# qcraftai/gedepth

Measured on AMD Instinct MI355X. Metric: training img/s (whole node), KITTI-shaped 352x1120 synthetic batches, higher is better.
Workload: dtype bf16; 1 GPU; depthformer_swint_v: DepthFormer-SwinT + GEDepth-Vanilla, 352x1120, 8 img/GPU, full train step; global_batch=8, parallelism=dp1, allreduce_dtype=fp32, layout=nhwc, window_attention=bf16 mfma, params=53516992, hip_graph=off

## Files before the change

gedepth_amd/csrc/conv3x3_wgrad.hip:

```cpp
#include "common.h"

#define WG_TH 8
#define WG_TW 32
#define WG_HALO ((WG_TH + 2) * (WG_TW + 2))
#define WG_PIX (WG_TH * WG_TW)
#define WG_DY_PIECES (WG_PIX * 8)
#define WG_X_PIECES (WG_HALO * 4)

template <int TAP0, int NTAP>
__device__ __forceinline__ void wg_tile_mfma(const bf16_t* dyh, const bf16_t* xt, ge_f32x16* acc) {
  ge_bf16x8 A[2], B[2][NTAP];
#define WG_RD(P) __builtin_shufflevector(__builtin_amdgcn_ds_read_tr16_b64_v4bf16(GE_LDS(ge_bf16x4, (P))), \
                                         __builtin_amdgcn_ds_read_tr16_b64_v4bf16(GE_LDS(ge_bf16x4, (P) + 4 * 32)), 0, 1, 2, 3, 4, 5, 6, 7)
#define WG_FRAGS(SET, KS)                                                                                   \
  {                                                                                                         \
    constexpr int row_ = (KS) >> 1, xh_ = ((KS) & 1) * 16;                                                  \
    A[SET] = WG_RD(dyh + (row_ * 32 + xh_) * 32);                                                           \
    _Pragma("unroll") for (int j = 0; j < NTAP; ++j) {                                                     \
      const int r_ = (TAP0 + j) / 3, s_ = (TAP0 + j) - 3 * r_;                                              \
      B[SET][j] = WG_RD(xt + ((row_ + r_) * (WG_TW + 2) + xh_ + s_) * 32);                                  \
    }                                                                                                       \
  }
#define WG_STEP(KS)                                                                                         \
  {                                                                                                         \
    if ((KS) < 15) WG_FRAGS(((KS) + 1) & 1, ((KS) + 1) & 15)                                                \
    __builtin_amdgcn_sched_barrier(0);                                                                      \
    _Pragma("unroll") for (int j = 0; j < NTAP; ++j)                                                       \
      acc[j] = __builtin_amdgcn_mfma_f32_32x32x16_bf16(A[(KS) & 1], B[(KS) & 1][j], acc[j], 0, 0, 0);       \
    __builtin_amdgcn_sched_barrier(0);                                                                      \
  }
  WG_FRAGS(0, 0)
  WG_STEP(0) WG_STEP(1) WG_STEP(2) WG_STEP(3) WG_STEP(4) WG_STEP(5) WG_STEP(6) WG_STEP(7)
  WG_STEP(8) WG_STEP(9) WG_STEP(10) WG_STEP(11) WG_STEP(12) WG_STEP(13) WG_STEP(14) WG_STEP(15)
#undef WG_STEP
#undef WG_FRAGS
#undef WG_RD
}

__global__ void __launch_bounds__(256, 2) conv3x3_wgrad_k(const bf16_t* __restrict__ x, const bf16_t* __restrict__ dy, float* __restrict__ dw, int N, int H,
                                                          int W, int Cin, int Cout, int tiles_x, int tiles_y, int ksplit) {
  __shared__ __attribute__((aligned(16))) bf16_t dy_t[2 * WG_PIX * 32];
  __shared__ __attribute__((aligned(16))) bf16_t x_t[WG_HALO * 32];
  const int tid = threadIdx.x, lane = tid & 63, wv = tid >> 6;
  const int c0 = blockIdx.x * 32, n0 = blockIdx.y * 64;
  const int mb = wv & 1, tap0 = (wv >> 1) ? 5 : 0, ntap = (wv >> 1) ? 4 : 5;
  ge_f32x16 acc[5];
#pragma unroll
  for (int t = 0; t < 5; ++t) acc[t] = 0.f;
  const int tr_pix = (lane >> 5) * 8 + ((lane & 15) >> 2), tr_col = ((lane >> 4) & 1) * 16 + (lane & 3) * 4;
  const int total_tiles = N * tiles_y * tiles_x;
  uint4 pd[8], px[6];
  const uint4 zero4 = make_uint4(0, 0, 0, 0);
  int dy_yx[8], dy_lds[8], x_yx[6], x_lds[6];
  const int dy_ch = n0 + (tid & 7) * 8, x_ch = c0 + (tid & 3) * 8;
#pragma unroll
  for (int i = 0; i < 8; ++i) {
    const int p = tid + i * 256, pix = p >> 3, part = p & 7;
    dy_yx[i] = ((pix >> 5) << 16) | (pix & 31);
    dy_lds[i] = ((part >> 2) * WG_PIX + pix) * 32 + (part & 3) * 8;
  }
#pragma unroll
  for (int i = 0; i < 6; ++i) {
    const int p = tid + i * 256, pix = p >> 2;
    const int iy = pix / (WG_TW + 2), ix = pix - iy * (WG_TW + 2);
    x_yx[i] = p < WG_X_PIECES ? ((iy << 16) | ix) : -1;
    x_lds[i] = (p >> 2) * 32 + (p & 3) * 8;
  }
  const bool dy_ch_ok = dy_ch < Cout;
#define WG_PREFETCH(T)                                                                                       \
  {                                                                                                          \
    const int t_ = __builtin_amdgcn_readfirstlane(T);                                                        \
    const int per_img = tiles_y * tiles_x;                                                                   \
    const int n_ = t_ / per_img, rem_ = t_ - n_ * per_img;                                                   \
    const int tyi = rem_ / tiles_x;                                                                          \
    const int ty0 = tyi * WG_TH, tx0 = (rem_ - tyi * tiles_x) * WG_TW;                                       \
    const bf16_t* dyn = dy + (long)n_ * H * W * Cout + dy_ch;                                                \
    const bf16_t* xn = x + (long)n_ * H * W * Cin + x_ch;                                                    \
    _Pragma("unroll") for (int i = 0; i < 8; ++i) {                                                         \
      const int gy = ty0 + (dy_yx[i] >> 16), gx = tx0 + (dy_yx[i] & 0xffff);                                 \
      pd[i] = zero4;                                                                                         \
      if (gy < H && gx < W && dy_ch_ok) pd[i] = *(const uint4*)(dyn + (gy * W + gx) * Cout);                 \
    }                                                                                                        \
    _Pragma("unroll") for (int i = 0; i < 6; ++i) {                                                         \
      const int gy = ty0 + (x_yx[i] >> 16) - 1, gx = tx0 + (x_yx[i] & 0xffff) - 1;                           \
      px[i] = zero4;                                                                                         \
      if (x_yx[i] >= 0 && gy >= 0 && gy < H && gx >= 0 && gx < W) px[i] = *(const uint4*)(xn + (gy * W + gx) * Cin); \
    }                                                                                                        \
  }
#define WG_PARK()                                                                                            \
  _Pragma("unroll") for (int i = 0; i < 8; ++i) *(uint4*)(dy_t + dy_lds[i]) = pd[i];                        \
  _Pragma("unroll") for (int i = 0; i < 6; ++i) {                                                           \
    if (x_yx[i] >= 0) *(uint4*)(x_t + x_lds[i]) = px[i];                                                     \
  }
  int t = blockIdx.z;
  if (t < total_tiles) {
    WG_PREFETCH(t)
    WG_PARK()
  }
  __syncthreads();
  for (; t < total_tiles; t += ksplit) {
    const bool more = t + ksplit < total_tiles;
    if (more) { WG_PREFETCH(t + ksplit) }
    const bf16_t* dyh = dy_t + mb * WG_PIX * 32 + tr_pix * 32 + tr_col;
    const bf16_t* xt = x_t + tr_pix * 32 + tr_col;
    if (wv >> 1) wg_tile_mfma<5, 4>(dyh, xt, acc);
    else wg_tile_mfma<0, 5>(dyh, xt, acc);
    __syncthreads();
    if (more) { WG_PARK() }
    __syncthreads();
  }
#undef WG_PREFETCH
#undef WG_PARK
  const int ci = c0 + (lane & 31);
#pragma unroll
  for (int j = 0; j < 5; ++j) {
    if (j < ntap) {
      const int tap = tap0 + j;
#pragma unroll
      for (int r = 0; r < 16; ++r) {
        const int co = n0 + mb * 32 + (r & 3) + 8 * (r >> 2) + 4 * (lane >> 5);
        if (co < Cout) atomicAdd(dw + ((long)co * 9 + tap) * Cin + ci, acc[j][r]);
      }
    }
  }
}

extern "C" int ge_conv3x3_nhwc_wgrad(const void* x, const void* dy, float* dw, int N, int H, int W, int Cin, int Cout, int dtype, void* stream) {
  if (!x || !dy || !dw || N < 0 || H <= 0 || W <= 0 || Cin <= 0 || Cout <= 0) return GE_ERR_BAD_ARG;
  if (dtype != GE_BF16 || Cin % 32 || Cout % 8 || (((uintptr_t)x | (uintptr_t)dy) & 15)) return GE_ERR_UNSUPPORTED;
  if (N == 0) return GE_OK;
  const int tiles_x = (W + WG_TW - 1) / WG_TW, tiles_y = (H + WG_TH - 1) / WG_TH;
  const long total = (long)N * tiles_y * tiles_x;
  if (total >= (1L << 31) || (long)H * W * std::max(Cin, Cout) >= (1L << 31)) return GE_ERR_UNSUPPORTED;
  const int blocks_out = (Cin / 32) * ((Cout + 63) / 64);
  const int cus = ge_cu_count();
  if (!cus) return GE_ERR_BAD_ARG;
  long ksplit = (2L * cus) / blocks_out;
  if (ksplit > total) ksplit = total;
  if (ksplit < 1) ksplit = 1;
  if (ksplit > 65535 || (Cout + 63) / 64 > 65535) return GE_ERR_UNSUPPORTED;
  const dim3 grid(Cin / 32, (Cout + 63) / 64, (unsigned)ksplit);
  conv3x3_wgrad_k<<<grid, 256, 0, ge_stream(stream)>>>((const bf16_t*)x, (const bf16_t*)dy, dw, N, H, W, Cin, Cout, tiles_x, tiles_y, (int)ksplit);
  GE_LAUNCH_CHECK();
  return GE_OK;
}
```

Baseline: 171.4 img/s.

## Rewrite conv3x3 wgrad with direct global-to-LDS DMA interleaved into MFMA loop

Replaces the register-staged prefetch/park wgrad kernel with a 512-thread kernel. Each block covers 64 input and 64 output channels and fills double-buffered LDS using global_load_lds_dwordx4, issued one slot per MFMA step so loads overlap compute. Work is split across waves by tap-role, blocks are remapped for XCD locality, and the per-class k-split is chosen from a cost table. This removes the VGPR staging and the second barrier, but adds large LDS use (160KB, one block per CU), inline asm, and more complex indexing. Only the conv3x3 weight gradient inside the full train step is affected.

```diff
diff --git a/gedepth_amd/csrc/conv3x3_wgrad.hip b/gedepth_amd/csrc/conv3x3_wgrad.hip
--- a/gedepth_amd/csrc/conv3x3_wgrad.hip
+++ b/gedepth_amd/csrc/conv3x3_wgrad.hip
@@ -4,11 +4,9 @@
 #define WG_TW 32
 #define WG_HALO ((WG_TH + 2) * (WG_TW + 2))
 #define WG_PIX (WG_TH * WG_TW)
-#define WG_DY_PIECES (WG_PIX * 8)
-#define WG_X_PIECES (WG_HALO * 4)
 
-template <int TAP0, int NTAP>
-__device__ __forceinline__ void wg_tile_mfma(const bf16_t* dyh, const bf16_t* xt, ge_f32x16* acc) {
+template <int TAP0, int NTAP, typename D>
+__device__ __forceinline__ void wg_tile_mfma(const bf16_t* dyh, const bf16_t* xt, ge_f32x16* acc, D&& dma) {
   ge_bf16x8 A[2], B[2][NTAP];
 #define WG_RD(P) __builtin_shufflevector(__builtin_amdgcn_ds_read_tr16_b64_v4bf16(GE_LDS(ge_bf16x4, (P))), \
                                          __builtin_amdgcn_ds_read_tr16_b64_v4bf16(GE_LDS(ge_bf16x4, (P) + 4 * 32)), 0, 1, 2, 3, 4, 5, 6, 7)
@@ -25,6 +23,7 @@
   {                                                                                                         \
     if ((KS) < 15) WG_FRAGS(((KS) + 1) & 1, ((KS) + 1) & 15)                                                \
     __builtin_amdgcn_sched_barrier(0);                                                                      \
+    dma(KS);                                                                                                \
     _Pragma("unroll") for (int j = 0; j < NTAP; ++j)                                                       \
       acc[j] = __builtin_amdgcn_mfma_f32_32x32x16_bf16(A[(KS) & 1], B[(KS) & 1][j], acc[j], 0, 0, 0);       \
     __builtin_amdgcn_sched_barrier(0);                                                                      \
@@ -37,81 +36,123 @@
 #undef WG_RD
 }
 
-__global__ void __launch_bounds__(256, 2) conv3x3_wgrad_k(const bf16_t* __restrict__ x, const bf16_t* __restrict__ dy, float* __restrict__ dw, int N, int H,
-                                                          int W, int Cin, int Cout, int tiles_x, int tiles_y, int ksplit) {
-  __shared__ __attribute__((aligned(16))) bf16_t dy_t[2 * WG_PIX * 32];
-  __shared__ __attribute__((aligned(16))) bf16_t x_t[WG_HALO * 32];
-  const int tid = threadIdx.x, lane = tid & 63, wv = tid >> 6;
-  const int c0 = blockIdx.x * 32, n0 = blockIdx.y * 64;
-  const int mb = wv & 1, tap0 = (wv >> 1) ? 5 : 0, ntap = (wv >> 1) ? 4 : 5;
+#define WD_XSLAB (22 * 1024)
+#define WD_XOFF (2 * WG_PIX * 64)
+#define WD_NPIECE (32 + 2 * 22)
+#define WD_SLOTS 10
+#define WD_BUF (80 * 1024)
+#ifndef WD_COST
+#define WD_COST {16, 11, 11, 7}
+#endif
+
+__device__ __attribute__((aligned(16))) uint32_t wd_zero16[4] = {0, 0, 0, 0};
+
+struct WdSplit { int k[4]; };
+
+__global__ void __launch_bounds__(512, 1) conv3x3_wgrad_dma_k(const bf16_t* __restrict__ x, const bf16_t* __restrict__ dy, float* __restrict__ dw, int N,
+                                                              int H, int W, int Cin, int Cout, int tiles_x, int tiles_y, WdSplit ks) {
+  __shared__ __attribute__((aligned(1024))) unsigned char smem[2 * WD_BUF];
+  const int tid = threadIdx.x, lane = tid & 63;
+  const int wv = __builtin_amdgcn_readfirstlane(tid >> 6);
+  const int chunks = Cin >> 5, pf = chunks >> 1, tail = chunks & 1;
+  const int cbs = (Cout + 63) >> 6, half = (Cout - 64 * (cbs - 1)) <= 32 ? 1 : 0, cf = cbs - half;
+  int b, pair, cb, ksplit;
+  {
+    const int per = gridDim.x >> 3, rem = gridDim.x & 7, xcd = blockIdx.x & 7;
+    b = xcd * per + (xcd < rem ? xcd : rem) + (blockIdx.x >> 3);
+  }
+  const int cnt0 = pf * cf * ks.k[0], cnt1 = pf * half * ks.k[1], cnt2 = tail * cf * ks.k[2];
+  if (b < cnt0) { ksplit = ks.k[0]; const int nb = pf * cf, z = b / nb, blk = b - z * nb; pair = blk / cf; cb = blk - pair * cf; b = z; }
+  else if ((b -= cnt0) < cnt1) { ksplit = ks.k[1]; const int z = b / pf; pair = b - z * pf; cb = cf; b = z; }
+  else if ((b -= cnt1) < cnt2) { ksplit = ks.k[2]; const int z = b / cf; cb = b - z * cf; pair = pf; b = z; }
+  else { b -= cnt2; ksplit = ks.k[3]; pair = pf; cb = cf; }
+  const int c0 = pair * 64, n0 = cb * 64;
+  const int nh = n0 + 32 < Cout ? 2 : 1, nc = c0 + 32 < Cin ? 2 : 1, units = nh * nc;
+  const int total_tiles = N * tiles_y * tiles_x, per_img = tiles_y * tiles_x;
+  int t = b;
+  if (t >= total_tiles) return;
+  int mb, ch, role;
+  if (units == 4) { ch = wv & 1; mb = wv >> 2; role = ((wv >> 1) & 1) ^ mb; }
+  else {
+    const int u = wv >> 2;
+    mb = nh == 2 ? u : 0; ch = nc == 2 ? u : 0;
+    role = u < units ? 2 + ((wv + 2 * u) & 3) : -1;
+  }
+  const int tap0 = role == 1 ? 5 : role == 3 ? 3 : role == 4 ? 5 : role == 5 ? 7 : 0;
+  const int ntap = role < 0 ? 0 : role == 0 ? 5 : role == 1 ? 4 : role == 2 ? 3 : 2;
   ge_f32x16 acc[5];
 #pragma unroll
-  for (int t = 0; t < 5; ++t) acc[t] = 0.f;
+  for (int j = 0; j < 5; ++j) acc[j] = 0.f;
+
+  int yx[WD_SLOTS];
+  const unsigned part16 = (lane & 3) * 16;
+#pragma unroll
+  for (int i = 0; i < WD_SLOTS; ++i) {
+    const int p = wv + 8 * i;
+    int v = -1;
+    if (p < 32) {
+      const int pix = (p & 15) * 16 + (lane >> 2);
+      if (n0 + (p >> 4) * 32 + (lane & 3) * 8 < Cout) v = (((pix >> 5) + 1) << 16) | ((pix & 31) + 1);
+    } else if (p < WD_NPIECE) {
+      const int q = p - 32, c = q >= 22 ? 1 : 0, hp = (q - 22 * c) * 16 + (lane >> 2);
+      if (hp < WG_HALO && c < nc) { const int iy = hp / (WG_TW + 2); v = (iy << 16) | (hp - iy * (WG_TW + 2)); }
+    }
+    yx[i] = v;
+  }
+  const unsigned char *s_dy = nullptr, *s_x = nullptr;
+  int s_ty0 = 0, s_tx0 = 0, s_buf = 0;
+  bool s_live = false;
+  auto aim = [&](int tt, bool live, int buf) {
+    const int n_ = tt / per_img, rem_ = tt - n_ * per_img, tyi = rem_ / tiles_x;
+    s_ty0 = tyi * WG_TH; s_tx0 = (rem_ - tyi * tiles_x) * WG_TW;
+    s_dy = (const unsigned char*)(dy + (long)n_ * H * W * Cout); s_x = (const unsigned char*)(x + (long)n_ * H * W * Cin);
+    s_live = live; s_buf = buf;
+  };
+  auto dma = [&](int i) {
+    if (i >= WD_SLOTS) return;
+    const int p = wv + 8 * i;
+    const bool isdy = p < 32;
+    const int C = isdy ? Cout : Cin;
+    const unsigned chb = (unsigned)(isdy ? n0 + (p >> 4) * 32 : c0 + (p >= 32 + 22 ? 32 : 0)) * 2u + part16;
+    const unsigned char* base = isdy ? s_dy : s_x;
+    const int v = yx[i], gy = s_ty0 + (v >> 16) - 1, gx = s_tx0 + (v & 0xffff) - 1;
+    const bool ok = s_live && v >= 0 && (unsigned)gy < (unsigned)H && (unsigned)gx < (unsigned)W;
+    const unsigned off = (unsigned)((gy * W + gx) * C) * 2u + chb;
+    const unsigned char* src = ok ? base + (size_t)off : (const unsigned char*)wd_zero16;
+    const unsigned ldst = (unsigned)(uintptr_t)GE_LDS(unsigned char, smem + s_buf * WD_BUF + p * 1024);
+    asm volatile("s_mov_b32 m0, %0\n\ts_nop 0\n\tglobal_load_lds_dwordx4 %1, off" :: "s"(ldst), "v"(src) : "memory", "m0");
+  };
   const int tr_pix = (lane >> 5) * 8 + ((lane & 15) >> 2), tr_col = ((lane >> 4) & 1) * 16 + (lane & 3) * 4;
-  const int total_tiles = N * tiles_y * tiles_x;
-  uint4 pd[8], px[6];
-  const uint4 zero4 = make_uint4(0, 0, 0, 0);
-  int dy_yx[8], dy_lds[8], x_yx[6], x_lds[6];
-  const int dy_ch = n0 + (tid & 7) * 8, x_ch = c0 + (tid & 3) * 8;
+  const int rd_dy = mb * WG_PIX * 64 + (tr_pix * 32 + tr_col) * 2, rd_x = WD_XOFF + ch * WD_XSLAB + (tr_pix * 32 + tr_col) * 2;
+
+  aim(t, true, 0);
 #pragma unroll
-  for (int i = 0; i < 8; ++i) {
-    const int p = tid + i * 256, pix = p >> 3, part = p & 7;
-    dy_yx[i] = ((pix >> 5) << 16) | (pix & 31);
-    dy_lds[i] = ((part >> 2) * WG_PIX + pix) * 32 + (part & 3) * 8;
+  for (int i = 0; i < WD_SLOTS; ++i) dma(i);
+  asm volatile("s_waitcnt vmcnt(0)" ::: "memory");
+  int buf = 0;
+  for (; t < total_tiles; t += ksplit) {
+    asm volatile("" ::: "memory");
+    __builtin_amdgcn_s_barrier();
+    asm volatile("" ::: "memory");
+    const bool more = t + ksplit < total_tiles;
+    aim(more ? t + ksplit : t, more, buf ^ 1);
+    const bf16_t* dyh = (const bf16_t*)(smem + buf * WD_BUF + rd_dy);
+    const bf16_t* xt = (const bf16_t*)(smem + buf * WD_BUF + rd_x);
+    switch (role) {
+      case 0: wg_tile_mfma<0, 5>(dyh, xt, acc, dma); break;
+      case 1: wg_tile_mfma<5, 4>(dyh, xt, acc, dma); break;
+      case 2: wg_tile_mfma<0, 3>(dyh, xt, acc, dma); break;
+      case 3: wg_tile_mfma<3, 2>(dyh, xt, acc, dma); break;
+      case 4: wg_tile_mfma<5, 2>(dyh, xt, acc, dma); break;
+      case 5: wg_tile_mfma<7, 2>(dyh, xt, acc, dma); break;
+      default:
+#pragma unroll
+        for (int i = 0; i < WD_SLOTS; ++i) dma(i);
+    }
+    asm volatile("s_waitcnt vmcnt(0)" ::: "memory");
+    buf ^= 1;
   }
-#pragma unroll
-  for (int i = 0; i < 6; ++i) {
-    const int p = tid + i * 256, pix = p >> 2;
-    const int iy = pix / (WG_TW + 2), ix = pix - iy * (WG_TW + 2);
-    x_yx[i] = p < WG_X_PIECES ? ((iy << 16) | ix) : -1;
-    x_lds[i] = (p >> 2) * 32 + (p & 3) * 8;
-  }
-  const bool dy_ch_ok = dy_ch < Cout;
-#define WG_PREFETCH(T)                                                                                       \
-  {                                                                                                          \
-    const int t_ = __builtin_amdgcn_readfirstlane(T);                                                        \
-    const int per_img = tiles_y * tiles_x;                                                                   \
-    const int n_ = t_ / per_img, rem_ = t_ - n_ * per_img;                                                   \
-    const int tyi = rem_ / tiles_x;                                                                          \
-    const int ty0 = tyi * WG_TH, tx0 = (rem_ - tyi * tiles_x) * WG_TW;                                       \
-    const bf16_t* dyn = dy + (long)n_ * H * W * Cout + dy_ch;                                                \
-    const bf16_t* xn = x + (long)n_ * H * W * Cin + x_ch;                                                    \
-    _Pragma("unroll") for (int i = 0; i < 8; ++i) {                                                         \
-      const int gy = ty0 + (dy_yx[i] >> 16), gx = tx0 + (dy_yx[i] & 0xffff);                                 \
-      pd[i] = zero4;                                                                                         \
-      if (gy < H && gx < W && dy_ch_ok) pd[i] = *(const uint4*)(dyn + (gy * W + gx) * Cout);                 \
-    }                                                                                                        \
-    _Pragma("unroll") for (int i = 0; i < 6; ++i) {                                                         \
-      const int gy = ty0 + (x_yx[i] >> 16) - 1, gx = tx0 + (x_yx[i] & 0xffff) - 1;                           \
-      px[i] = zero4;                                                                                         \
-      if (x_yx[i] >= 0 && gy >= 0 && gy < H && gx >= 0 && gx < W) px[i] = *(const uint4*)(xn + (gy * W + gx) * Cin); \
-    }                                                                                                        \
-  }
-#define WG_PARK()                                                                                            \
-  _Pragma("unroll") for (int i = 0; i < 8; ++i) *(uint4*)(dy_t + dy_lds[i]) = pd[i];                        \
-  _Pragma("unroll") for (int i = 0; i < 6; ++i) {                                                           \
-    if (x_yx[i] >= 0) *(uint4*)(x_t + x_lds[i]) = px[i];                                                     \
-  }
-  int t = blockIdx.z;
-  if (t < total_tiles) {
-    WG_PREFETCH(t)
-    WG_PARK()
-  }
-  __syncthreads();
-  for (; t < total_tiles; t += ksplit) {
-    const bool more = t + ksplit < total_tiles;
-    if (more) { WG_PREFETCH(t + ksplit) }
-    const bf16_t* dyh = dy_t + mb * WG_PIX * 32 + tr_pix * 32 + tr_col;
-    const bf16_t* xt = x_t + tr_pix * 32 + tr_col;
-    if (wv >> 1) wg_tile_mfma<5, 4>(dyh, xt, acc);
-    else wg_tile_mfma<0, 5>(dyh, xt, acc);
-    __syncthreads();
-    if (more) { WG_PARK() }
-    __syncthreads();
-  }
-#undef WG_PREFETCH
-#undef WG_PARK
-  const int ci = c0 + (lane & 31);
+  const int ci = c0 + ch * 32 + (lane & 31);
 #pragma unroll
   for (int j = 0; j < 5; ++j) {
     if (j < ntap) {
@@ -132,15 +173,24 @@
   const int tiles_x = (W + WG_TW - 1) / WG_TW, tiles_y = (H + WG_TH - 1) / WG_TH;
   const long total = (long)N * tiles_y * tiles_x;
   if (total >= (1L << 31) || (long)H * W * std::max(Cin, Cout) >= (1L << 31)) return GE_ERR_UNSUPPORTED;
-  const int blocks_out = (Cin / 32) * ((Cout + 63) / 64);
   const int cus = ge_cu_count();
   if (!cus) return GE_ERR_BAD_ARG;
-  long ksplit = (2L * cus) / blocks_out;
-  if (ksplit > total) ksplit = total;
-  if (ksplit < 1) ksplit = 1;
-  if (ksplit > 65535 || (Cout + 63) / 64 > 65535) return GE_ERR_UNSUPPORTED;
-  const dim3 grid(Cin / 32, (Cout + 63) / 64, (unsigned)ksplit);
-  conv3x3_wgrad_k<<<grid, 256, 0, ge_stream(stream)>>>((const bf16_t*)x, (const bf16_t*)dy, dw, N, H, W, Cin, Cout, tiles_x, tiles_y, (int)ksplit);
+  if ((Cout + 63) / 64 > 65535) return GE_ERR_UNSUPPORTED;
+  const long chunks = Cin / 32, pf = chunks / 2, tail = chunks & 1, cbs = (Cout + 63) / 64, half = Cout - 64 * (cbs - 1) <= 32, cf = cbs - half;
+  const long nblk[4] = {pf * cf, pf * half, tail * cf, tail * half};
+  const int cost[4] = WD_COST;
+  long all = 0, grid = 0;
+  for (int c = 0; c < 4; ++c) all += nblk[c] * cost[c];
+  WdSplit ks;
+  for (int c = 0; c < 4; ++c) {
+    long k = (long)cus * cost[c] / all;
+    if (k > total) k = total;
+    if (k < 1) k = 1;
+    ks.k[c] = (int)k;
+    grid += nblk[c] * k;
+  }
+  if (grid >= (1L << 31)) return GE_ERR_UNSUPPORTED;
+  conv3x3_wgrad_dma_k<<<dim3((unsigned)grid), 512, 0, ge_stream(stream)>>>((const bf16_t*)x, (const bf16_t*)dy, dw, N, H, W, Cin, Cout, tiles_x, tiles_y, ks);
   GE_LAUNCH_CHECK();
   return GE_OK;
 }
```

Result: no change. 172.6 img/s, median of 6 (+0.7%).
